# gbonneau-hardent/smallz4

Hardware: AMD Instinct MI355X
Metric: input MB/s at -9 optimal parse; output-byte diff vs smallz4 (must be 0) (higher is better)
Workload: dtype u8

## Files before the change

smallz4_amd/csrc/sz4_host.cpp:

```cpp
#include <hip/hip_runtime.h>

#include <algorithm>
#include <chrono>
#include <mutex>
#include <cstdio>
#include <atomic>
#include <cstring>
#include <string>
#include <new>
#include <vector>

#include "../../include/smallz4_amd.h"
#include "sz4_internal.h"
#include "sz4_mem.h"
#include "sz4_plan.h"

using namespace sz4;

namespace {

constexpr uint64_t kPad = 64;
constexpr uint64_t kBatchChunkDefault = 448ull << 20;
constexpr uint64_t kScratchPerByte = 50;
constexpr uint64_t kPieceFloor = 16ull << 20;
// ... 85 lines not shown
  PipeArgs a{};
  a.in = in;
  a.blocks = blocks.as<Block>();
  a.nblocks = (uint32_t)plan.blocks.size();
  a.segs = segs.as<Segment>();
  a.nsegs = (uint32_t)plan.segs.size();
  a.dpSegs = dpSegs.as<DpSeg>();
  a.ndp = (uint32_t)plan.dp.size();
  a.maxDpCount = plan.maxDpCount;
  a.walkSegs = walkSegs.as<uint2>();
  a.nwalk = (uint32_t)plan.walk.size();
  a.maxChain = maxChain;
  a.iv = iv.as<Interval>();
  a.ivCount = ivCount.as<uint32_t>();
  a.mlen = mlen.as<uint32_t>();
  a.mdist = mdist.as<uint16_t>();
  a.sel = sel();
  a.cost = cost.as<uint32_t>();
  a.reach = reach.as<uint32_t>();
  a.longFlag = longFlag.as<uint32_t>();
  a.longBits = longBits.as<uint32_t>();
  a.segLong = segLong.as<uint32_t>();
  a.segTail = segTail.as<uint64_t>();
  a.rank = rank.as<uint32_t>();
  const Plan::WorkOffsets& off = plan.off;
  a.elemA = work.as<uint2>();
  a.elemB = work_at<uint2>(off.elemB);
  a.rmqUp = work_at<uint32_t>(off.rmqUp);
  a.rmqDown = work_at<uint32_t>(off.rmqDown);
  a.dpSide = work_at<uint2>(off.side);
  a.dpRec = dpRec.as<uint4>();
  a.segState = segState.as<uint4>();
  a.lazySlots = work_at<uint32_t>(off.lazy);
  a.walkSlots = work_at<uint32_t>(off.walk);
  a.walkState = walkState.as<uint4>();
  a.tokens = work_at<Token>(off.tok);
  a.ntok = ntok.as<uint32_t>();
  a.blockBytes = blockBytes.as<uint32_t>();
  a.offsets = offsets.as<uint64_t>();
  a.status = status.as<int>();
  a.ldsWindow = plan.ldsWindow;
  a.out = out;
  a.headerLen = hdrLen;
  a.chosen = maxChain > (uint32_t)kGreedyMax ? a.sel : a.mlen;
  return a;
}

hipError_t Pipe::upload_plan(hipStream_t s) const
{
  hipError_t e = hipSuccess;
  (e = hipMemcpyAsync(blocks.p, plan.blocks.data(), plan.blocks.size() * sizeof(Block), hipMemcpyHostToDevice, s)) ||
      (e = hipMemcpyAsync(segs.p, plan.segs.data(), plan.segs.size() * sizeof(Segment), hipMemcpyHostToDevice, s)) ||
      (e = hipMemcpyAsync(dpSegs.p, plan.dp.data(), plan.dp.size() * sizeof(DpSeg), hipMemcpyHostToDevice, s)) ||
      (e = hipMemcpyAsync(walkSegs.p, plan.walk.data(), plan.walk.size() * sizeof(uint2), hipMemcpyHostToDevice, s));
  return e;
}

}

struct sz4_ctx {
  int device = 0;
  std::string err;
  bool timing = false;
  hipEvent_t ev[kStages + 1] = {};
  float stageMs[kStages] = {};
  uint32_t lastBlocks = 0;
  int stopAfter = 0;
  uint32_t lastChain = 0;

// ... 1703 lines not shown
```

smallz4_amd/csrc/sz4_internal.h:

```cpp
#pragma once
#include <stdint.h>

#include <hip/hip_runtime.h>

namespace sz4 {

constexpr int kMinMatch = 4;
constexpr int kTailNoMatch = 12;
constexpr int kTailLiterals = 5;
constexpr uint32_t kWindow = 65535;
constexpr uint32_t kSameLetter = 19 + 255 * 256;
constexpr int kGreedyMax = 3;
constexpr int kLazyMax = 6;
constexpr uint32_t kHashMul = 48271;
constexpr int kHashBits = 20;
constexpr uint64_t kNone = ~0ull;
constexpr uint32_t kRmqLen = 274;
constexpr uint32_t kFlagRmq = 1;
constexpr uint32_t kFlagRun = 2;
constexpr int kStages = 6;

constexpr int kStPrepRound = 2;
constexpr int kStInvariant = 4;

// ... 9 lines not shown
  uint32_t walkFirst;
  uint32_t walkCount;
  uint32_t dpSize;
  uint32_t pad;
};
constexpr uint32_t kNoBlock = 0xFFFFFFFFu;
constexpr uint32_t kBlkLegacy = 1;

struct Segment {
  uint64_t w0, s0, s1;
  uint64_t elemOff;
  uint64_t rankOff;
  uint32_t block;
  uint32_t pad;
};

struct Interval {
  uint64_t lo, hi;
  uint64_t a;
  uint64_t La;
};
constexpr uint32_t kMaxIv = 136;

struct DpSeg {
  uint32_t block;
  uint32_t k;
  uint32_t lo, hi;
};
inline uint32_t dp_segment_size(uint64_t n) { return n <= 65536 ? 4096u : 8192u; }
constexpr uint32_t kMaxDpSegs = 2048;

constexpr uint32_t kWalkSeg = 4096;
constexpr uint32_t kWalkCap = kWalkSeg / 4 + 2;

struct Token {
  uint32_t litFrom, lits, mlen, dist;
};
constexpr uint32_t kTokLast = 0x80000000u;

constexpr uint32_t kFindLds = 65536 + 16;
constexpr uint32_t find_lds_bytes() { return kFindLds; }
constexpr uint32_t kDpSide = 512;
constexpr uint32_t kDpSideKeys = kDpSide + 256;
constexpr uint32_t kDpSideStride = kDpSide + kDpSideKeys;
constexpr uint32_t dp_side_positions() { return kDpSideStride; }
constexpr uint32_t kLazyCap = 1400;
constexpr uint32_t lazy_slots_per_walk() { return 2 * kLazyCap; }

struct PipeArgs {
  const uint8_t* in;
  const Block* blocks;
  uint32_t nblocks;
  const Segment* segs;
  uint32_t nsegs;
  const DpSeg* dpSegs;
  uint32_t ndp;
  uint32_t maxDpCount;
  const uint2* walkSegs;
  uint32_t nwalk;
  uint32_t maxChain;
  Interval* iv;
  uint32_t* ivCount;
  uint32_t* mlen;
  uint16_t* mdist;
  uint32_t* sel;
  uint32_t* cost;
  uint32_t* reach;
  uint32_t* longFlag;
  uint32_t* longBits;
  uint32_t* segLong;
  uint64_t* segTail;
  uint32_t* rank;
  uint2* elemA;
  uint2* elemB;
  uint32_t* rmqUp;
  uint32_t* rmqDown;
  uint2* dpSide;
  uint4* dpRec;
  uint4* segState;
  uint32_t* lazySlots;
  uint32_t* walkSlots;
  uint4* walkState;
  Token* tokens;
  uint32_t* ntok;
  uint32_t* blockBytes;
  uint64_t* offsets;
  int* status;
  bool ldsWindow;
  uint8_t* out;
  uint64_t headerLen;
  const uint32_t* chosen;
};
void launch_runs(const PipeArgs& a, hipStream_t s);
void launch_find(int pass, const PipeArgs& a, hipStream_t s);
constexpr uint64_t kBlockMaxDict = 4ull << 20;
constexpr uint64_t kBlockMaxLegacy = 8ull << 20;
struct DictArgs : PipeArgs {
  const Block* hBlocks;
  uint32_t dictBack, cont, shift, low0;
  int legacy;
  uint32_t* last;
  uint16_t *prevH, *prevX, *ph, *pe;
  uint64_t *keysA, *keysB;
  void* temp;
  uint64_t tempBytes;
  uint32_t* lzMasks;
  uint64_t* scBits;
  uint2* runTab;
  uint32_t* runFlag;
  bool buildRuns;
  bool guess;
};
void launch_dict(const DictArgs& a, hipStream_t s);
uint64_t dict_sort_keys_max();
uint64_t dict_sort_temp_bytes();
uint64_t dict_sc_bits_bytes(uint32_t nb, uint64_t maxBlock);
// ... 102 lines not shown
```

smallz4_amd/csrc/sz4_kernels.hip:

```cpp
#include <hip/hip_runtime.h>
#include <stdint.h>
#include <stdlib.h>

#include <type_traits>

#include "sz4_internal.h"
#include "sz4_device.h"

#ifndef SZ4_SKIP_SHIFT
#define SZ4_SKIP_SHIFT 0
#endif
#ifndef SZ4_SKIP_BCAST
#define SZ4_SKIP_BCAST 0
#endif
#ifndef SZ4_SKIP_SEARCH
#define SZ4_SKIP_SEARCH 0
#endif
#ifndef SZ4_DIAG
#define SZ4_DIAG 0
#endif
#if SZ4_DIAG == 3
#define SZ4_D3(...) __VA_ARGS__
#else
#define SZ4_D3(...)
#endif
#if SZ4_DIAG == 5
#define SZ4_D5(...) __VA_ARGS__
#else
#define SZ4_D5(...)
#endif
#if SZ4_DIAG == 7
#define SZ4_D7(...) __VA_ARGS__
#else
#define SZ4_D7(...)
#endif

namespace sz4 {


__device__ __forceinline__ uint32_t lload4(const uint32_t* w, uint32_t off)
// ... 4797 lines not shown
        deltaTab[k] = convDelta;
        aboveTab[k] = 0;
        if (!done) segState[B.dpFirst + k] = make_uint4(lits, litBump, 0u, 0u);
      }
      prevV = convDelta;
      prevConv = (uint32_t)conv;
      prevDone = done;
      __syncthreads();
      prevKeyLim = convBlk[k];
    }
  }
  SZ4_D7(
  if (!kPar && lane == 0) {
    const uint64_t dt = __builtin_readcyclecounter() - d7t0;
    atomicAdd((unsigned long long*)&sz4_diag[0], (unsigned long long)d7Serial);
    atomicAdd((unsigned long long*)&sz4_diag[1], (unsigned long long)d7Closed);
    atomicAdd((unsigned long long*)&sz4_diag[2], (unsigned long long)d7Lit);
    atomicAdd((unsigned long long*)&sz4_diag[3], (unsigned long long)d7Segs);
    atomicMax((unsigned long long*)&sz4_diag[4], (unsigned long long)d7Serial);
    atomicAdd((unsigned long long*)&sz4_diag[5], (unsigned long long)dt);
    atomicMax((unsigned long long*)&sz4_diag[6], (unsigned long long)dt);
    atomicAdd((unsigned long long*)&sz4_diag[7], 1ull);
    if (rmq) atomicAdd((unsigned long long*)&sz4_diag[8], 1ull);
    for (int q = 0; q < 4; q++) atomicAdd((unsigned long long*)&sz4_diag[9 + q], (unsigned long long)d7Tk[q]);
  }
  )
}



__global__ __launch_bounds__(64 * kWalkWaves) void k_walk(const Block* __restrict__ blocks,
                                                          const uint2* __restrict__ walkSegs, uint32_t nwalk,
                                                          const uint32_t* __restrict__ chosen,
                                                          uint32_t* __restrict__ slotsAll, uint4* __restrict__ state,
                                                          int* __restrict__ status)
{
  const uint32_t wave = (uint32_t)__builtin_amdgcn_readfirstlane((int)(threadIdx.x >> 6));
  const uint32_t idx = blockIdx.x * kWalkWaves + wave;
  if (idx >= nwalk) return;
  const uint32_t lane = threadIdx.x & 63;
  const uint2 ws = walkSegs[idx];
  const Block B = blocks[ws.x];
  if (ws.y >= B.walkCount) return;
  const uint32_t n = (uint32_t)(B.end - B.start);
  const uint32_t* L = chosen + B.start;
  uint32_t* slots = slotsAll + (uint64_t)idx * (2 * kWalkCap) + kWalkCap;
  const uint32_t a = ws.y * kWalkSeg;
  const uint32_t aNext = a + kWalkSeg < n ? a + kWalkSeg : n;

  auto ldw = [&](uint32_t b) -> uint32_t {
    const uint32_t i = b + lane;
    return L[i < n ? i : n - 1u];
  };
  uint32_t wbase = a, e = 0, m = 0, exitPos = aNext;
  uint32_t wL = ldw(a), nL = ldw(a + 64);
  while (true) {
    const uint32_t lim = aNext - wbase < 64u ? aNext - wbase : 64u;
    const uint32_t len = wbase + lane < n && wL > 1u ? wL : 1u;
    const uint64_t mm = __ballot(len > 1u && lane >= e && lane < lim);
    uint32_t next, lastLen = 1;
    if (mm == 0) {
      next = wbase + lim;
    } else {
      const uint32_t x = wave_path(lane + len < 64u ? lane + len : 64u, e, lane);
      const bool rec = x == lane && len > 1u && lane < lim;
      const uint64_t rb = __ballot(rec);
      const uint32_t cnt = (uint32_t)__builtin_popcountll(rb);
      if (m + cnt > kWalkCap) {
        if (lane == 0) atomicOr(status, kStInvariant);
        break;
      }
      if (rec) slots[m + __builtin_amdgcn_mbcnt_hi((uint32_t)(rb >> 32), __builtin_amdgcn_mbcnt_lo((uint32_t)rb, 0u))] = wbase + lane;
      m += cnt;
      const uint32_t p = rdlane(x, lim - 1u);
      lastLen = rdlane(len, p);
      next = wbase + p + lastLen;
    }
    if (next >= aNext) {
      exitPos = lastLen > 1u ? next : aNext;
      break;
    }
    const uint32_t nb = next & ~63u;
    wL = nb == wbase + 64u ? nL : ldw(nb);
    nL = ldw(nb + 64u);
    wbase = nb;
    e = next & 63u;
  }
  if (lane == 0) state[idx] = make_uint4(kWalkCap, kWalkCap + m, exitPos, 0u);
}

struct WalkRepair {
  const uint32_t* L;
  const uint32_t* slots;
  uint32_t lane;
  __device__ __forceinline__ uint4 run(uint32_t* fix, uint32_t a, uint32_t aNext, uint4 st, uint32_t entry, int* status) const
  {
    const uint32_t m = st.y - kWalkCap;
    if (entry == a) return make_uint4(st.x, 0u, st.z, entry);
    if (entry >= aNext) return make_uint4(st.y, 0u, entry, entry);
    auto first_at = [&](uint32_t from, uint32_t p) -> uint32_t {
      for (uint32_t b = from; b < m; b += 64) {
        const uint64_t ge = __ballot(b + lane < m && slots[kWalkCap + b + lane] >= p);
        if (ge) return b + (uint32_t)__builtin_ctzll(ge);
      }
      return m;
    };
    auto inside = [&](uint32_t i, uint32_t q) -> bool {
      if (i == 0) return false;
      const uint32_t pj = slots[kWalkCap + i - 1];
      return pj + L[pj] > q;
    };
    uint32_t i = first_at(0, entry);
    if (!inside(i, entry)) return make_uint4(kWalkCap + i, 0u, st.z, entry);
    uint32_t q = entry, f = 0;
    bool merged = false;
    while (q < aNext) {
      const uint32_t lq = L[q];
      if (lq > 1u) {
        if (f >= kWalkCap) {
          if (lane == 0) atomicOr(status, kStInvariant);
          break;
        }
        if (lane == 0) fix[f] = q;
        f++;
        q += lq;
      } else {
        q++;
      }
      i = first_at(i, q);
      if (q < aNext && !inside(i, q)) {
        merged = true;
        break;
      }
    }
    const uint32_t iMerge = merged ? i : m;
    return make_uint4(kWalkCap + iMerge - f, f, merged ? st.z : q, entry);
  }
};

__global__ __launch_bounds__(64 * kWalkWaves) void k_walk_fix_spec(const Block* __restrict__ blocks,
                                                                   const uint2* __restrict__ walkSegs, uint32_t nwalk,
                                                                   const uint32_t* __restrict__ chosen,
                                                                   uint32_t* __restrict__ slotsAll,
                                                                   const uint4* __restrict__ state, uint4* __restrict__ rec,
                                                                   int* __restrict__ status)
{
  __shared__ uint32_t fixAll[kWalkWaves][kWalkCap];
  const uint32_t wave = (uint32_t)__builtin_amdgcn_readfirstlane((int)(threadIdx.x >> 6));
  const uint32_t idx = blockIdx.x * kWalkWaves + wave;
  if (idx >= nwalk) return;
  const uint2 ws = walkSegs[idx];
  if (ws.y == 0) return;
  const uint32_t lane = threadIdx.x & 63;
  const Block B = blocks[ws.x];
  if (ws.y >= B.walkCount) return;
  const uint32_t n = (uint32_t)(B.end - B.start);
  const uint32_t a = ws.y * kWalkSeg, aNext = a + kWalkSeg < n ? a + kWalkSeg : n;
  uint32_t* slots = slotsAll + (uint64_t)idx * (2 * kWalkCap);
  const WalkRepair W{chosen + B.start, slots, lane};
  uint32_t* fix = fixAll[wave];
  const uint4 r = W.run(fix, a, aNext, state[idx], state[idx - 1].z, status);
  __builtin_amdgcn_wave_barrier();
  for (uint32_t t = lane; t < r.y; t += 64) slots[t] = fix[t];
  if (lane == 0) rec[idx] = r;
}

__global__ __launch_bounds__(64) void k_walk_fix_commit(const Block* __restrict__ blocks, const uint32_t* __restrict__ chosen,
                                                        uint32_t* __restrict__ slotsAll,
                                                        uint4* __restrict__ state, const uint4* __restrict__ rec,
                                                        int* __restrict__ status)
{
  __shared__ uint32_t fix[kWalkCap];
  const Block B = blocks[blockIdx.x];
  if (B.walkCount < 2) return;
  const uint32_t lane = threadIdx.x;
  const uint32_t n = (uint32_t)(B.end - B.start);
  const uint32_t* L = chosen + B.start;
  uint32_t T = state[B.walkFirst].z;
  for (uint32_t k0 = 1; k0 < B.walkCount; k0 += 64) {
    const uint32_t cnt = B.walkCount - k0 < 64u ? B.walkCount - k0 : 64u;
    const uint32_t idxL = B.walkFirst + k0 + lane;
    const uint4 r = lane < cnt ? rec[idxL] : make_uint4(0, 0, 0, 0);
    uint32_t cur = 0;
    while (cur < cnt) {
      uint32_t prevExit = __shfl_up(r.z, 1, 64);
      if (lane == cur) prevExit = T;
      const uint64_t bad = __ballot(lane >= cur && lane < cnt && r.w != prevExit);
      const uint32_t js = bad ? (uint32_t)__builtin_ctzll(bad) : cnt;
      if (lane >= cur && lane < js) {
        uint32_t* slots = slotsAll + (uint64_t)idxL * (2 * kWalkCap);
        for (uint32_t t = r.y; t-- > 0;) slots[r.x + t] = slots[t];
        uint32_t* s32 = reinterpret_cast<uint32_t*>(state + idxL);
        s32[0] = r.x;
        s32[2] = r.z;
      }
      if (js == cnt) {
        T = rdlane(r.z, cnt - 1u);
        break;
      }
      const uint32_t idx = B.walkFirst + k0 + js;
      const uint32_t a = (k0 + js) * kWalkSeg, aNext = a + kWalkSeg < n ? a + kWalkSeg : n;
      uint32_t* slots = slotsAll + (uint64_t)idx * (2 * kWalkCap);
      const WalkRepair W{L, slots, lane};
      const uint4 st = state[idx];
      const uint4 rr = W.run(fix, a, aNext, st, rdlane(prevExit, js), status);
      __syncthreads();
      for (uint32_t t = lane; t < rr.y; t += 64) slots[rr.x + t] = fix[t];
      if (lane == 0) state[idx] = make_uint4(rr.x, st.y, rr.z, 0u);
      __syncthreads();
      T = rr.z;
      cur = js + 1;
    }
  }
}

__device__ __forceinline__ uint64_t token_bytes(uint64_t lits, uint32_t mlen, bool last)
{
  uint64_t b = 1 + lits + (lits >= 15 ? (lits - 15) / 255 + 1 : 0);
  if (!last) {
    const int64_t mcode = (int64_t)mlen - kMinMatch;
    b += 2 + (mcode >= 15 ? (uint64_t)(mcode - 15) / 255 + 1 : 0);
  }
  return b;
}

__global__ __launch_bounds__(1024) void k_scan(const uint32_t* __restrict__ blockBytes, uint32_t nblocks,
                                               uint64_t* __restrict__ offsets)
{
  __shared__ uint64_t s_carry;
  __shared__ uint32_t s_w[16];
  const uint32_t tid = threadIdx.x, lane = tid & 63, wave = tid >> 6;
  if (tid == 0) s_carry = 0;
  __syncthreads();
  for (uint32_t base = 0; base < nblocks; base += 1024) {
    const uint32_t i = base + tid;
    const uint32_t v = i < nblocks ? (blockBytes[i] & 0x7FFFFFFFu) : 0u;
    const uint32_t incl = wave_incl_scan_add(v);
    if (lane == 63) s_w[wave] = incl;
    __syncthreads();
    uint64_t pre = s_carry;
    for (uint32_t w = 0; w < wave; w++) pre += s_w[w];
    if (i < nblocks) offsets[i] = pre + incl - v;
    __syncthreads();
    if (tid == 1023) s_carry = pre + incl;
    __syncthreads();
  }
  if (tid == 0) offsets[nblocks] = s_carry;
}

constexpr uint64_t kOwnLits = 64;

constexpr int kAsmThreads = 1024;
constexpr int kSegWaves = 4;

__device__ __forceinline__ uint32_t wave_sum_u32(uint32_t v)
{
#pragma unroll
  for (int d = 32; d >= 1; d >>= 1) v += __shfl_xor(v, d, 64);
  return v;
}

__global__ __launch_bounds__(kAsmThreads) void k_seg_scan(const Block* __restrict__ blocks, const uint32_t* __restrict__ chosen,
                                                          const uint32_t* __restrict__ slotsAll,
                                                          const uint4* __restrict__ state, uint4* __restrict__ info)
{
  __shared__ uint32_t s_sum[kAsmThreads / 64], s_max[kAsmThreads / 64];
  const Block B = blocks[blockIdx.x];
  if (B.start == B.end) return;
  const uint32_t* L = chosen + B.start;
  const uint32_t tid = threadIdx.x, lane = tid & 63, wave = tid >> 6;
  uint32_t carrySum = 0, carryMax = 0;
  for (uint32_t k0 = 0; k0 < B.walkCount; k0 += kAsmThreads) {
    const uint32_t k = k0 + tid;
    const bool valid = k < B.walkCount;
    const uint32_t idx = B.walkFirst + k;
    uint32_t cnt = 0, lastEnd = 0;
    if (valid) {
      const uint4 st = state[idx];
      cnt = st.y - st.x;
      if (cnt) {
        const uint32_t p = slotsAll[(uint64_t)idx * (2 * kWalkCap) + st.y - 1];
        lastEnd = p + L[p];
      }
    }
    const uint32_t incS = wave_incl_scan_add(cnt), incM = wave_incl_scan_max(lastEnd);
    uint32_t prevM = __shfl_up(incM, 1, 64);
    if (lane == 0) prevM = 0;
    if (lane == 63) {
      s_sum[wave] = incS;
      s_max[wave] = incM;
    }
    __syncthreads();
    uint32_t preS = carrySum, preM = carryMax;
    for (uint32_t w = 0; w < wave; w++) {
      preS += s_sum[w];
      preM = s_max[w] > preM ? s_max[w] : preM;
    }
    if (valid) info[idx] = make_uint4(preS + incS - cnt, prevM > preM ? prevM : preM, 0u, 0u);
    for (uint32_t w = 0; w < kAsmThreads / 64; w++) {
      carrySum += s_sum[w];
      carryMax = s_max[w] > carryMax ? s_max[w] : carryMax;
    }
    __syncthreads();
  }
}

__global__ __launch_bounds__(64 * kSegWaves) void k_seg_tokens(const Block* __restrict__ blocks, const uint2* __restrict__ walkSegs,
                                                              uint32_t nwalk, const uint32_t* __restrict__ chosen,
                                                              const uint16_t* __restrict__ mdist,
                                                              const uint32_t* __restrict__ slotsAll, const uint4* __restrict__ state,
                                                              uint4* __restrict__ info, Token* __restrict__ tokAll,
                                                              uint2* __restrict__ blockTail)
{
  const uint32_t wave = (uint32_t)__builtin_amdgcn_readfirstlane((int)(threadIdx.x >> 6));
  const uint32_t idx = blockIdx.x * kSegWaves + wave;
  if (idx >= nwalk) return;
  const uint32_t lane = threadIdx.x & 63;
  const uint2 ws = walkSegs[idx];
  const Block B = blocks[ws.x];
  if (ws.y >= B.walkCount) return;
  const uint32_t n = (uint32_t)(B.end - B.start);
  const uint32_t* L = chosen + B.start;
  const uint16_t* D = mdist + B.start;
  const uint4 st = state[idx];
  const uint4 inf = info[idx];
  const uint32_t m = st.y - st.x;
  const uint32_t* slots = slotsAll + (uint64_t)idx * (2 * kWalkCap);
  Token* tok = tokAll + B.tokOff + inf.x;
  uint32_t carryEnd = inf.y, bytes = 0;
  uint32_t pN = lane < m ? slots[st.x + lane] : 0u;
  uint32_t LN = lane < m ? L[pN] : 0u, DN = lane < m ? (uint32_t)D[pN] : 0u;
  uint32_t pNN = 64u + lane < m ? slots[st.x + 64u + lane] : 0u;
  for (uint32_t c0 = 0; c0 < m; c0 += 64) {
    const uint32_t t = c0 + lane;
    const bool valid = t < m;
    uint32_t p, Lm, Dm;
    asm volatile("v_mov_b32 %0, %1" : "=v"(p) : "v"(pN));
    asm volatile("v_mov_b32 %0, %1" : "=v"(Lm) : "v"(LN));
    asm volatile("v_mov_b32 %0, %1" : "=v"(Dm) : "v"(DN));
    pN = pNN;
    LN = t + 64u < m ? L[pN] : 0u;
    DN = t + 64u < m ? (uint32_t)D[pN] : 0u;
    pNN = t + 128u < m ? slots[st.x + t + 128u] : 0u;
    const uint32_t end = p + Lm;
    uint32_t prev = __shfl_up(end, 1, 64);
    if (lane == 0) prev = carryEnd;
    uint32_t sz = 0;
    if (valid) {
      const uint32_t lits = p - prev;
      tok[t] = Token{lits ? prev : 0u, lits, Lm, Dm};
      sz = (uint32_t)token_bytes(lits, Lm, false);
    }
    bytes += wave_sum_u32(sz);
    carryEnd = rdlane(end, m - c0 < 64 ? m - c0 - 1 : 63);
  }
  if (lane == 0) info[idx].z = bytes;
  if (ws.y + 1 == B.walkCount && lane == 0) {
    const uint32_t M = inf.x + m;
    tokAll[B.tokOff + M] = Token{carryEnd, n - carryEnd, 0u, kTokLast};
    blockTail[ws.x] = make_uint2(M, (uint32_t)token_bytes(n - carryEnd, 0, true));
  }
}

__global__ __launch_bounds__(kAsmThreads) void k_block_bytes(const Block* __restrict__ blocks, uint32_t maxChain,
                                                             uint4* __restrict__ info, const uint2* __restrict__ blockTail,
                                                             uint32_t* __restrict__ ntokOut, uint32_t* __restrict__ blockBytes,
                                                             int* __restrict__ status)
{
  __shared__ uint32_t s_sum[kAsmThreads / 64];
  const Block B = blocks[blockIdx.x];
  const uint32_t tid = threadIdx.x, lane = tid & 63, wave = tid >> 6;
  const uint64_t n = B.end - B.start;
  if (n == 0) {
    if (tid == 0) ntokOut[blockIdx.x] = 0u, blockBytes[blockIdx.x] = 0u;
    return;
  }
  const bool stored = maxChain == 0;
  const bool legacy = (B.flags & kBlkLegacy) != 0;
  uint64_t enc = 0;
  uint32_t ntok = 0;
  if (!stored) {
    uint32_t carry = 0;
    for (uint32_t k0 = 0; k0 < B.walkCount; k0 += kAsmThreads) {
      const uint32_t k = k0 + tid;
      const bool valid = k < B.walkCount;
      const uint32_t idx = B.walkFirst + k;
      const uint32_t b = valid ? info[idx].z : 0u;
      const uint32_t inc = wave_incl_scan_add(b);
      if (lane == 63) s_sum[wave] = inc;
      __syncthreads();
      uint32_t pre = carry;
      for (uint32_t w = 0; w < wave; w++) pre += s_sum[w];
      if (valid) info[idx].w = pre + inc - b;
      for (uint32_t w = 0; w < kAsmThreads / 64; w++) carry += s_sum[w];
      __syncthreads();
    }
    const uint2 tail = blockTail[blockIdx.x];
    enc = (uint64_t)carry + tail.y;
    ntok = tail.x + 1;
  }
  const bool useEnc = (enc < n && !stored) || legacy;
  const uint32_t bytes = (uint32_t)(useEnc ? enc : n);
  if (tid == 0 && (ntok > n / 2 + 4 || (useEnc ? enc : n) >= 0x7FFFFFFBull)) atomicOr(status, kStInvariant);
  if (tid == 0) {
    ntokOut[blockIdx.x] = useEnc ? ntok : 0u;
    blockBytes[blockIdx.x] = (useEnc ? 0u : 0x80000000u) | (bytes + 4u);
  }
}

__global__ __launch_bounds__(64 * kSegWaves) void k_write_seg(const uint8_t* __restrict__ in, const Block* __restrict__ blocks,
                                                             const uint2* __restrict__ walkSegs, uint32_t nwalk,
                                                             const uint4* __restrict__ state, const uint4* __restrict__ info,
                                                             const Token* __restrict__ tokAll, const uint32_t* __restrict__ ntokAll,
                                                             const uint32_t* __restrict__ blockBytes,
                                                             const uint64_t* __restrict__ offsets, uint8_t* __restrict__ out,
                                                             uint64_t headerLen)
{
  __shared__ uint32_t s_ld[kSegWaves][64], s_ls[kSegWaves][64], s_ll[kSegWaves][64];
  const uint32_t wave = (uint32_t)__builtin_amdgcn_readfirstlane((int)(threadIdx.x >> 6));
  const uint32_t idx = blockIdx.x * kSegWaves + wave;
  if (idx >= nwalk) return;
  const uint32_t lane = threadIdx.x & 63;
  const uint2 ws = walkSegs[idx];
  const Block B = blocks[ws.x];
  if (ws.y >= B.walkCount) return;
  const uint64_t n = B.end - B.start;
  const uint32_t bb = blockBytes[ws.x];
  const bool raw = (bb & 0x80000000u) != 0;
  uint8_t* dst = out + headerLen + offsets[ws.x];
  if (ws.y == 0 && lane == 0) {
    const uint32_t word = ((bb & 0x7FFFFFFFu) - 4u) | (raw ? 0x80000000u : 0u);
    dst[0] = (uint8_t)word;
    dst[1] = (uint8_t)(word >> 8);
    dst[2] = (uint8_t)(word >> 16);
    dst[3] = (uint8_t)(word >> 24);
  }
  dst += 4;
  const uint8_t* src = in + B.start;
  if (raw) {
    const uint64_t lo = (uint64_t)ws.y * kWalkSeg, hi = lo + kWalkSeg < n ? lo + kWalkSeg : n;
    for (uint64_t j = lo + lane; j < hi; j += 64) dst[j] = src[j];
    return;
  }
  if (ntokAll[ws.x] == 0) return;
  const uint4 st = state[idx], inf = info[idx];
  const uint32_t count = (st.y - st.x) + (ws.y + 1 == B.walkCount ? 1u : 0u);
  const Token* tok = tokAll + B.tokOff + inf.x;
  uint64_t carry = inf.w;
  for (uint32_t c0 = 0; c0 < count; c0 += 64) {
    const uint32_t t = c0 + lane;
    const bool valid = t < count;
    Token T{0, 0, 0, 0};
    uint64_t sz = 0;
    bool last = false;
    if (valid) {
      T = tok[t];
      last = (T.dist & kTokLast) != 0;
      sz = token_bytes(T.lits, T.mlen, last);
    }
    uint64_t incl = sz;
#pragma unroll
    for (int d = 1; d < 64; d <<= 1) {
      const uint64_t o = __shfl_up(incl, d, 64);
      if (lane >= (uint32_t)d) incl += o;
    }
    const uint64_t off = carry + incl - sz;
    carry += __shfl(incl, 63, 64);
    bool isLong = false;
    if (valid) {
      uint8_t* o = dst + off;
      const int64_t mcode = last ? 0 : (int64_t)T.mlen - kMinMatch;
      const uint8_t tk = (uint8_t)(mcode < 15 ? mcode : 15);
      const uint64_t lits = T.lits;
      if (lits < 15) {
        *o++ = (uint8_t)(tk | (lits << 4));
      } else {
        *o++ = (uint8_t)(tk | 0xF0);
        uint64_t v = lits - 15;
        while (v >= 255) { *o++ = 255; v -= 255; }
        *o++ = (uint8_t)v;
      }
      if (lits <= kOwnLits) {
        for (uint32_t k = 0; k < (uint32_t)lits; k += 8) {
          const uint64_t a = (uint64_t)T.litFrom + k;
          const uint32_t nk = (uint32_t)lits - k < 8u ? (uint32_t)lits - k : 8u;
          const uintptr_t ab = reinterpret_cast<uintptr_t>(src + a);
          if (a >= 4u && a + 12u <= n) {
            const uint32_t* wp = reinterpret_cast<const uint32_t*>(ab & ~(uintptr_t)3);
            const uint32_t w0 = wp[0], w1 = wp[1], w2 = wp[2];
            const uint32_t sh = (uint32_t)(ab & 3u);
            const uint32_t v0 = __builtin_amdgcn_alignbyte(w1, w0, sh), v1 = __builtin_amdgcn_alignbyte(w2, w1, sh);
#pragma unroll
// ... 109 lines not shown
  hipMemsetAsync(firstBad, 0xFF, (size_t)a.nblocks * 4, s);
  hipLaunchKernelGGL(k_lazy_check, walks, walkBlock, 0, s, a.in, a.blocks, a.walkSegs, a.nwalk, a.iv, a.ivCount, a.longFlag,
                     a.mlen, a.mdist, a.lazySlots, a.walkState, firstBad);
  hipLaunchKernelGGL(k_lazy_correct, dim3(a.nblocks), dim3(64), 0, s, a.blocks, a.iv, a.ivCount, a.mlen, firstBad,
                     a.status);
}

void launch_parse(const PipeArgs& a, hipStream_t s)
{
  if (!a.nblocks) return;
  if (a.maxChain <= (uint32_t)kGreedyMax || !a.ndp) return;
  const dim3 specGrid((a.ndp + kSpecWaves - 1) / kSpecWaves), specBlock(64 * kSpecWaves);
  hipLaunchKernelGGL(k_dp_spec_lean, specGrid, specBlock, 0, s, a.blocks, a.dpSegs, a.ndp, a.mlen, a.mdist, a.cost, a.sel,
                     a.reach, a.segState, a.longFlag, a.rmqUp, a.rmqDown);
  hipLaunchKernelGGL(k_dp_spec_rmq, specGrid, specBlock, 0, s, a.blocks, a.dpSegs, a.ndp, a.mlen, a.mdist, a.cost, a.sel,
                     a.reach, a.segState, a.longFlag, a.rmqUp, a.rmqDown);
  hipLaunchKernelGGL(k_dp_fix<true>, dim3(a.ndp), dim3(64), 0, s, a.blocks, a.dpSegs, a.ndp, a.mlen, a.mdist, a.cost, a.sel,
                     a.reach, a.segState, a.longFlag, a.rmqUp, a.rmqDown, a.dpSide, a.dpRec, 0u);
  const uint32_t tab = a.maxDpCount < 1u ? 1u : a.maxDpCount > kMaxDpSegs ? kMaxDpSegs : a.maxDpCount;
  hipLaunchKernelGGL(k_dp_fix<false>, dim3(a.nblocks), dim3(64), 4 * tab * sizeof(uint32_t), s, a.blocks, a.dpSegs, a.ndp,
                     a.mlen, a.mdist, a.cost, a.sel, a.reach, a.segState, a.longFlag, a.rmqUp, a.rmqDown, a.dpSide, a.dpRec,
                     tab);
}

void launch_emit(const PipeArgs& a, hipStream_t s)
{
  if (!a.nblocks) return;
  const bool walk = a.maxChain > 0 && a.nwalk;
  const dim3 walks((a.nwalk + kWalkWaves - 1) / kWalkWaves), walkBlock(64 * kWalkWaves);
  const dim3 segGrid((a.nwalk + kSegWaves - 1) / kSegWaves), segBlock(64 * kSegWaves);
  uint4* info = reinterpret_cast<uint4*>(a.reach);
  uint2* blockTail = reinterpret_cast<uint2*>(info + a.nwalk);
  if (walk) {
    hipLaunchKernelGGL(k_walk, walks, walkBlock, 0, s, a.blocks, a.walkSegs, a.nwalk, a.chosen, a.walkSlots, a.walkState,
                       a.status);
    hipLaunchKernelGGL(k_walk_fix_spec, walks, walkBlock, 0, s, a.blocks, a.walkSegs, a.nwalk, a.chosen, a.walkSlots,
                       a.walkState, info, a.status);
    hipLaunchKernelGGL(k_walk_fix_commit, dim3(a.nblocks), dim3(64), 0, s, a.blocks, a.chosen, a.walkSlots, a.walkState,
                       info, a.status);
    hipLaunchKernelGGL(k_seg_scan, dim3(a.nblocks), dim3(kAsmThreads), 0, s, a.blocks, a.chosen, a.walkSlots, a.walkState,
                       info);
    hipLaunchKernelGGL(k_seg_tokens, segGrid, segBlock, 0, s, a.blocks, a.walkSegs, a.nwalk, a.chosen, a.mdist, a.walkSlots,
                       a.walkState, info, a.tokens, blockTail);
  }
  hipLaunchKernelGGL(k_block_bytes, dim3(a.nblocks), dim3(kAsmThreads), 0, s, a.blocks, a.maxChain, info, blockTail, a.ntok,
                     a.blockBytes, a.status);
  hipLaunchKernelGGL(k_scan, dim3(1), dim3(1024), 0, s, a.blockBytes, a.nblocks, a.offsets);
  if (a.nwalk)
    hipLaunchKernelGGL(k_write_seg, segGrid, segBlock, 0, s, a.in, a.blocks, a.walkSegs, a.nwalk, a.walkState, info, a.tokens,
                       a.ntok, a.blockBytes, a.offsets, a.out, a.headerLen);
}

}
```

smallz4_amd/csrc/sz4_plan.cpp:

```cpp
#include "sz4_plan.h"

#include <stdlib.h>

#include <algorithm>

namespace sz4 {

Block independent_block(uint64_t start, uint64_t end, uint32_t flags)
{
  Block B{};
  B.start = start;
  B.end = end;
  B.low = start;
  B.cut = kNone;
  B.prev = kNoBlock;
  B.flags = flags;
  return B;
}

bool Plan::begin(const PlanKey& k)
{
  if (k == key) return false;
  key = PlanKey{};
  blocks.clear();
// ... 57 lines not shown
    }
    B.dpSize = (uint32_t)seg;
    for (uint64_t hi = top, i = 0;; hi -= seg, i++) {
      const uint64_t lo = hi + 1 >= seg ? hi + 1 - seg : 0;
      dp.push_back(DpSeg{b, (uint32_t)i, (uint32_t)lo, (uint32_t)hi});
      B.dpCount++;
      if (lo == 0) break;
    }
    maxDpCount = std::max(maxDpCount, B.dpCount);
  }
  ldsWindow = true;
  for (const Segment& S : segs) {
    const Block& B = blocks[S.block];
    if ((B.end - S.w0 + 8 + 3) / 4 * 4 > find_lds_bytes()) ldsWindow = false;
  }
  key = k;
}

uint64_t Plan::work_layout(uint64_t stagedBytes)
{
  auto al = [](uint64_t b) { return (b + 255) & ~255ull; };
  const uint64_t nb = blocks.size();
  const uint64_t elem = al(elemTotal * sizeof(uint2) + 64);
  off.elemB = elem;
  const uint64_t findEnd = 2 * elem;
  const uint64_t selBytes = al(stagedBytes * 4 + 64), rmq = al((stagedBytes + nb + 8) * 4);
  off.rmqUp = selBytes;
  off.rmqDown = selBytes + rmq;
  off.side = selBytes + 2 * rmq;
  const uint64_t parseEnd = off.side + al(dp.size() * dp_side_positions() * sizeof(uint2) + 64);
  off.lazy = selBytes;
  const uint64_t lazyEnd = off.lazy + al(walk.size() * lazy_slots_per_walk() * 4ull + 64);
  off.tok = selBytes;
  off.walk = off.tok + al(tokTotal * sizeof(Token) + 64);
  const uint64_t emitEnd = off.walk + al(walk.size() * 2 * kWalkCap * 4 + 64);
  return std::max(std::max(findEnd, parseEnd), std::max(lazyEnd, emitEnd));
}

void Plan::build_uniform(uint64_t len, uint32_t blockSize)
{
  const PlanKey k{PlanKey::kUniform, len, blockSize};
  if (!begin(k)) return;
  for (uint64_t st = 0; st < len; st += blockSize)
    blocks.push_back(independent_block(st, std::min<uint64_t>(st + blockSize, len)));
  finish_plan(k);
}

void Plan::build_stream(uint64_t pre, uint64_t n, bool first, int legacy, bool dictMode)
{
  const PlanKey k{PlanKey::kStream, 0, 0, pre, n, first, legacy, dictMode};
  if (!begin(k)) return;
  const uint64_t bs = legacy ? kBlockMaxLegacy : kBlockMaxDict;
  for (uint64_t st = 0; st < n; st += bs) {
    Block B = independent_block(pre + st, pre + std::min(st + bs, n), legacy ? kBlkLegacy : 0);
    if (!legacy && !(st == 0 && first)) {
      B.low = B.start - kWindow;
      B.cut = B.start - kTailNoMatch;
      B.prev = st == 0 ? kNoBlock - 1 : (uint32_t)blocks.size() - 1;
    }
    blocks.push_back(B);
  }
  const uint32_t nb = (uint32_t)blocks.size();
  if (nb && blocks[0].prev == kNoBlock - 1) blocks[0].prev = nb;
  finish_plan(k);
}

uint64_t Plan::build_ragged(const std::vector<uint64_t>& sizes)
// ... 58 lines not shown
```

Before: 15610.

## Pack match records into 64-bit walk slots and drop the token array

Walk slots now hold packed 64-bit records (position, length, distance) instead of bare positions, so later stages no longer gather L[p] and D[p] through a position indirection. The separate Token array and its write in the segment pass are removed, and the writer rebuilds literal spans from neighbouring records with shuffles. The spec-fix kernel writes repairs straight into global slots instead of LDS, and slots are laid out per block via tokOff with per-segment caps. This trades wider slot storage and a 24-bit position/length limit for fewer global writes and random reads.

```diff
diff --git a/smallz4_amd/csrc/sz4_host.cpp b/smallz4_amd/csrc/sz4_host.cpp
--- a/smallz4_amd/csrc/sz4_host.cpp
+++ b/smallz4_amd/csrc/sz4_host.cpp
@@ -141,9 +141,8 @@
   a.dpRec = dpRec.as<uint4>();
   a.segState = segState.as<uint4>();
   a.lazySlots = work_at<uint32_t>(off.lazy);
-  a.walkSlots = work_at<uint32_t>(off.walk);
+  a.walkSlots = work_at<uint64_t>(off.tok);
   a.walkState = walkState.as<uint4>();
-  a.tokens = work_at<Token>(off.tok);
   a.ntok = ntok.as<uint32_t>();
   a.blockBytes = blockBytes.as<uint32_t>();
   a.offsets = offsets.as<uint64_t>();
diff --git a/smallz4_amd/csrc/sz4_internal.h b/smallz4_amd/csrc/sz4_internal.h
--- a/smallz4_amd/csrc/sz4_internal.h
+++ b/smallz4_amd/csrc/sz4_internal.h
@@ -65,11 +65,8 @@
 
 constexpr uint32_t kWalkSeg = 4096;
 constexpr uint32_t kWalkCap = kWalkSeg / 4 + 2;
-
-struct Token {
-  uint32_t litFrom, lits, mlen, dist;
-};
-constexpr uint32_t kTokLast = 0x80000000u;
+constexpr uint32_t walk_cap(uint32_t r) { return r / 4 + 2 < kWalkCap ? r / 4 + 2 : kWalkCap; }
+constexpr uint64_t walk_slot_first(uint64_t tokOff, uint32_t k) { return 2 * tokOff + (uint64_t)k * kWalkSeg; }
 
 constexpr uint32_t kFindLds = 65536 + 16;
 constexpr uint32_t find_lds_bytes() { return kFindLds; }
@@ -112,9 +109,8 @@
   uint4* dpRec;
   uint4* segState;
   uint32_t* lazySlots;
-  uint32_t* walkSlots;
+  uint64_t* walkSlots;
   uint4* walkState;
-  Token* tokens;
   uint32_t* ntok;
   uint32_t* blockBytes;
   uint64_t* offsets;
diff --git a/smallz4_amd/csrc/sz4_kernels.hip b/smallz4_amd/csrc/sz4_kernels.hip
--- a/smallz4_amd/csrc/sz4_kernels.hip
+++ b/smallz4_amd/csrc/sz4_kernels.hip
@@ -6,6 +6,7 @@
 
 #include "sz4_internal.h"
 #include "sz4_device.h"
+#include "sz4_match_rec.h"
 
 #ifndef SZ4_SKIP_SHIFT
 #define SZ4_SKIP_SHIFT 0
@@ -4869,7 +4870,8 @@
 __global__ __launch_bounds__(64 * kWalkWaves) void k_walk(const Block* __restrict__ blocks,
                                                           const uint2* __restrict__ walkSegs, uint32_t nwalk,
                                                           const uint32_t* __restrict__ chosen,
-                                                          uint32_t* __restrict__ slotsAll, uint4* __restrict__ state,
+                                                          const uint16_t* __restrict__ mdist,
+                                                          uint64_t* __restrict__ slotsAll, uint4* __restrict__ state,
                                                           int* __restrict__ status)
 {
   const uint32_t wave = (uint32_t)__builtin_amdgcn_readfirstlane((int)(threadIdx.x >> 6));
@@ -4881,16 +4883,23 @@
   if (ws.y >= B.walkCount) return;
   const uint32_t n = (uint32_t)(B.end - B.start);
   const uint32_t* L = chosen + B.start;
-  uint32_t* slots = slotsAll + (uint64_t)idx * (2 * kWalkCap) + kWalkCap;
+  const uint16_t* D = mdist + B.start;
   const uint32_t a = ws.y * kWalkSeg;
   const uint32_t aNext = a + kWalkSeg < n ? a + kWalkSeg : n;
+  const uint32_t cap = walk_cap(aNext - a);
+  uint64_t* slots = slotsAll + walk_slot_first(B.tokOff, ws.y) + cap;
 
   auto ldw = [&](uint32_t b) -> uint32_t {
     const uint32_t i = b + lane;
     return L[i < n ? i : n - 1u];
   };
+  auto ldd = [&](uint32_t b) -> uint32_t {
+    const uint32_t i = b + lane;
+    return D[i < n ? i : n - 1u];
+  };
   uint32_t wbase = a, e = 0, m = 0, exitPos = aNext;
   uint32_t wL = ldw(a), nL = ldw(a + 64);
+  uint32_t wD = ldd(a), nD = ldd(a + 64);
   while (true) {
     const uint32_t lim = aNext - wbase < 64u ? aNext - wbase : 64u;
     const uint32_t len = wbase + lane < n && wL > 1u ? wL : 1u;
@@ -4903,11 +4912,13 @@
       const bool rec = x == lane && len > 1u && lane < lim;
       const uint64_t rb = __ballot(rec);
       const uint32_t cnt = (uint32_t)__builtin_popcountll(rb);
-      if (m + cnt > kWalkCap) {
+      if (m + cnt > cap) {
         if (lane == 0) atomicOr(status, kStInvariant);
         break;
       }
-      if (rec) slots[m + __builtin_amdgcn_mbcnt_hi((uint32_t)(rb >> 32), __builtin_amdgcn_mbcnt_lo((uint32_t)rb, 0u))] = wbase + lane;
+      if (rec)
+        slots[m + __builtin_amdgcn_mbcnt_hi((uint32_t)(rb >> 32), __builtin_amdgcn_mbcnt_lo((uint32_t)rb, 0u))] =
+            mrec_pack(wbase + lane, len, wD);
       m += cnt;
       const uint32_t p = rdlane(x, lim - 1u);
       lastLen = rdlane(len, p);
@@ -4919,46 +4930,49 @@
     }
     const uint32_t nb = next & ~63u;
     wL = nb == wbase + 64u ? nL : ldw(nb);
+    wD = nb == wbase + 64u ? nD : ldd(nb);
     nL = ldw(nb + 64u);
+    nD = ldd(nb + 64u);
     wbase = nb;
     e = next & 63u;
   }
-  if (lane == 0) state[idx] = make_uint4(kWalkCap, kWalkCap + m, exitPos, 0u);
+  if (lane == 0) state[idx] = make_uint4(cap, cap + m, exitPos, 0u);
 }
 
 struct WalkRepair {
   const uint32_t* L;
-  const uint32_t* slots;
+  const uint16_t* D;
+  const uint64_t* slots;
   uint32_t lane;
-  __device__ __forceinline__ uint4 run(uint32_t* fix, uint32_t a, uint32_t aNext, uint4 st, uint32_t entry, int* status) const
+  uint32_t cap;
+  __device__ __forceinline__ uint4 run(uint64_t* fix, uint32_t a, uint32_t aNext, uint4 st, uint32_t entry, int* status) const
   {
-    const uint32_t m = st.y - kWalkCap;
+    const uint32_t m = st.y - cap;
     if (entry == a) return make_uint4(st.x, 0u, st.z, entry);
     if (entry >= aNext) return make_uint4(st.y, 0u, entry, entry);
     auto first_at = [&](uint32_t from, uint32_t p) -> uint32_t {
       for (uint32_t b = from; b < m; b += 64) {
-        const uint64_t ge = __ballot(b + lane < m && slots[kWalkCap + b + lane] >= p);
+        const uint64_t ge = __ballot(b + lane < m && mrec_pos(slots[cap + b + lane]) >= p);
         if (ge) return b + (uint32_t)__builtin_ctzll(ge);
       }
       return m;
     };
     auto inside = [&](uint32_t i, uint32_t q) -> bool {
       if (i == 0) return false;
-      const uint32_t pj = slots[kWalkCap + i - 1];
-      return pj + L[pj] > q;
+      return mrec_end(slots[cap + i - 1]) > q;
     };
     uint32_t i = first_at(0, entry);
-    if (!inside(i, entry)) return make_uint4(kWalkCap + i, 0u, st.z, entry);
+    if (!inside(i, entry)) return make_uint4(cap + i, 0u, st.z, entry);
     uint32_t q = entry, f = 0;
     bool merged = false;
     while (q < aNext) {
       const uint32_t lq = L[q];
       if (lq > 1u) {
-        if (f >= kWalkCap) {
+        if (f >= cap) {
           if (lane == 0) atomicOr(status, kStInvariant);
           break;
         }
-        if (lane == 0) fix[f] = q;
+        if (lane == 0) fix[f] = mrec_pack(q, lq, D[q]);
         f++;
         q += lq;
       } else {
@@ -4971,18 +4985,18 @@
       }
     }
     const uint32_t iMerge = merged ? i : m;
-    return make_uint4(kWalkCap + iMerge - f, f, merged ? st.z : q, entry);
+    return make_uint4(cap + iMerge - f, f, merged ? st.z : q, entry);
   }
 };
 
 __global__ __launch_bounds__(64 * kWalkWaves) void k_walk_fix_spec(const Block* __restrict__ blocks,
                                                                    const uint2* __restrict__ walkSegs, uint32_t nwalk,
                                                                    const uint32_t* __restrict__ chosen,
-                                                                   uint32_t* __restrict__ slotsAll,
+                                                                   const uint16_t* __restrict__ mdist,
+                                                                   uint64_t* __restrict__ slotsAll,
                                                                    const uint4* __restrict__ state, uint4* __restrict__ rec,
                                                                    int* __restrict__ status)
 {
-  __shared__ uint32_t fixAll[kWalkWaves][kWalkCap];
   const uint32_t wave = (uint32_t)__builtin_amdgcn_readfirstlane((int)(threadIdx.x >> 6));
   const uint32_t idx = blockIdx.x * kWalkWaves + wave;
   if (idx >= nwalk) return;
@@ -4993,26 +5007,25 @@
   if (ws.y >= B.walkCount) return;
   const uint32_t n = (uint32_t)(B.end - B.start);
   const uint32_t a = ws.y * kWalkSeg, aNext = a + kWalkSeg < n ? a + kWalkSeg : n;
-  uint32_t* slots = slotsAll + (uint64_t)idx * (2 * kWalkCap);
-  const WalkRepair W{chosen + B.start, slots, lane};
-  uint32_t* fix = fixAll[wave];
-  const uint4 r = W.run(fix, a, aNext, state[idx], state[idx - 1].z, status);
-  __builtin_amdgcn_wave_barrier();
-  for (uint32_t t = lane; t < r.y; t += 64) slots[t] = fix[t];
+  uint64_t* slots = slotsAll + walk_slot_first(B.tokOff, ws.y);
+  const WalkRepair W{chosen + B.start, mdist + B.start, slots, lane, walk_cap(aNext - a)};
+  const uint4 r = W.run(slots, a, aNext, state[idx], state[idx - 1].z, status);
   if (lane == 0) rec[idx] = r;
 }
 
 __global__ __launch_bounds__(64) void k_walk_fix_commit(const Block* __restrict__ blocks, const uint32_t* __restrict__ chosen,
-                                                        uint32_t* __restrict__ slotsAll,
+                                                        const uint16_t* __restrict__ mdist,
+                                                        uint64_t* __restrict__ slotsAll,
                                                         uint4* __restrict__ state, const uint4* __restrict__ rec,
                                                         int* __restrict__ status)
 {
-  __shared__ uint32_t fix[kWalkCap];
+  __shared__ uint64_t fix[kWalkCap];
   const Block B = blocks[blockIdx.x];
   if (B.walkCount < 2) return;
   const uint32_t lane = threadIdx.x;
   const uint32_t n = (uint32_t)(B.end - B.start);
   const uint32_t* L = chosen + B.start;
+  const uint16_t* D = mdist + B.start;
   uint32_t T = state[B.walkFirst].z;
   for (uint32_t k0 = 1; k0 < B.walkCount; k0 += 64) {
     const uint32_t cnt = B.walkCount - k0 < 64u ? B.walkCount - k0 : 64u;
@@ -5025,7 +5038,7 @@
       const uint64_t bad = __ballot(lane >= cur && lane < cnt && r.w != prevExit);
       const uint32_t js = bad ? (uint32_t)__builtin_ctzll(bad) : cnt;
       if (lane >= cur && lane < js) {
-        uint32_t* slots = slotsAll + (uint64_t)idxL * (2 * kWalkCap);
+        uint64_t* slots = slotsAll + walk_slot_first(B.tokOff, k0 + lane);
         for (uint32_t t = r.y; t-- > 0;) slots[r.x + t] = slots[t];
         uint32_t* s32 = reinterpret_cast<uint32_t*>(state + idxL);
         s32[0] = r.x;
@@ -5037,8 +5050,8 @@
       }
       const uint32_t idx = B.walkFirst + k0 + js;
       const uint32_t a = (k0 + js) * kWalkSeg, aNext = a + kWalkSeg < n ? a + kWalkSeg : n;
-      uint32_t* slots = slotsAll + (uint64_t)idx * (2 * kWalkCap);
-      const WalkRepair W{L, slots, lane};
+      uint64_t* slots = slotsAll + walk_slot_first(B.tokOff, k0 + js);
+      const WalkRepair W{L, D, slots, lane, walk_cap(aNext - a)};
       const uint4 st = state[idx];
       const uint4 rr = W.run(fix, a, aNext, st, rdlane(prevExit, js), status);
       __syncthreads();
@@ -5049,16 +5062,6 @@
       cur = js + 1;
     }
   }
-}
-
-__device__ __forceinline__ uint64_t token_bytes(uint64_t lits, uint32_t mlen, bool last)
-{
-  uint64_t b = 1 + lits + (lits >= 15 ? (lits - 15) / 255 + 1 : 0);
-  if (!last) {
-    const int64_t mcode = (int64_t)mlen - kMinMatch;
-    b += 2 + (mcode >= 15 ? (uint64_t)(mcode - 15) / 255 + 1 : 0);
-  }
-  return b;
 }
 
 __global__ __launch_bounds__(1024) void k_scan(const uint32_t* __restrict__ blockBytes, uint32_t nblocks,
@@ -5097,14 +5100,13 @@
   return v;
 }
 
-__global__ __launch_bounds__(kAsmThreads) void k_seg_scan(const Block* __restrict__ blocks, const uint32_t* __restrict__ chosen,
-                                                          const uint32_t* __restrict__ slotsAll,
+__global__ __launch_bounds__(kAsmThreads) void k_seg_scan(const Block* __restrict__ blocks,
+                                                          const uint64_t* __restrict__ slotsAll,
                                                           const uint4* __restrict__ state, uint4* __restrict__ info)
 {
   __shared__ uint32_t s_sum[kAsmThreads / 64], s_max[kAsmThreads / 64];
   const Block B = blocks[blockIdx.x];
   if (B.start == B.end) return;
-  const uint32_t* L = chosen + B.start;
   const uint32_t tid = threadIdx.x, lane = tid & 63, wave = tid >> 6;
   uint32_t carrySum = 0, carryMax = 0;
   for (uint32_t k0 = 0; k0 < B.walkCount; k0 += kAsmThreads) {
@@ -5115,10 +5117,7 @@
     if (valid) {
       const uint4 st = state[idx];
       cnt = st.y - st.x;
-      if (cnt) {
-        const uint32_t p = slotsAll[(uint64_t)idx * (2 * kWalkCap) + st.y - 1];
-        lastEnd = p + L[p];
-      }
+      if (cnt) lastEnd = mrec_end(slotsAll[walk_slot_first(B.tokOff, k) + st.y - 1]);
     }
     const uint32_t incS = wave_incl_scan_add(cnt), incM = wave_incl_scan_max(lastEnd);
     uint32_t prevM = __shfl_up(incM, 1, 64);
@@ -5142,12 +5141,10 @@
   }
 }
 
-__global__ __launch_bounds__(64 * kSegWaves) void k_seg_tokens(const Block* __restrict__ blocks, const uint2* __restrict__ walkSegs,
-                                                              uint32_t nwalk, const uint32_t* __restrict__ chosen,
-                                                              const uint16_t* __restrict__ mdist,
-                                                              const uint32_t* __restrict__ slotsAll, const uint4* __restrict__ state,
-                                                              uint4* __restrict__ info, Token* __restrict__ tokAll,
-                                                              uint2* __restrict__ blockTail)
+__global__ __launch_bounds__(64 * kSegWaves) void k_seg_sizes(const Block* __restrict__ blocks, const uint2* __restrict__ walkSegs,
+                                                             uint32_t nwalk, const uint64_t* __restrict__ slotsAll,
+                                                             const uint4* __restrict__ state, uint4* __restrict__ info,
+                                                             uint2* __restrict__ blockTail)
 {
   const uint32_t wave = (uint32_t)__builtin_amdgcn_readfirstlane((int)(threadIdx.x >> 6));
   const uint32_t idx = blockIdx.x * kSegWaves + wave;
@@ -5157,45 +5154,26 @@
   const Block B = blocks[ws.x];
   if (ws.y >= B.walkCount) return;
   const uint32_t n = (uint32_t)(B.end - B.start);
-  const uint32_t* L = chosen + B.start;
-  const uint16_t* D = mdist + B.start;
   const uint4 st = state[idx];
   const uint4 inf = info[idx];
   const uint32_t m = st.y - st.x;
-  const uint32_t* slots = slotsAll + (uint64_t)idx * (2 * kWalkCap);
-  Token* tok = tokAll + B.tokOff + inf.x;
+  const uint64_t* recs = slotsAll + walk_slot_first(B.tokOff, ws.y) + st.x;
   uint32_t carryEnd = inf.y, bytes = 0;
-  uint32_t pN = lane < m ? slots[st.x + lane] : 0u;
-  uint32_t LN = lane < m ? L[pN] : 0u, DN = lane < m ? (uint32_t)D[pN] : 0u;
-  uint32_t pNN = 64u + lane < m ? slots[st.x + 64u + lane] : 0u;
+  uint64_t rN = lane < m ? recs[lane] : 0ull;
   for (uint32_t c0 = 0; c0 < m; c0 += 64) {
     const uint32_t t = c0 + lane;
-    const bool valid = t < m;
-    uint32_t p, Lm, Dm;
-    asm volatile("v_mov_b32 %0, %1" : "=v"(p) : "v"(pN));
-    asm volatile("v_mov_b32 %0, %1" : "=v"(Lm) : "v"(LN));
-    asm volatile("v_mov_b32 %0, %1" : "=v"(Dm) : "v"(DN));
-    pN = pNN;
-    LN = t + 64u < m ? L[pN] : 0u;
-    DN = t + 64u < m ? (uint32_t)D[pN] : 0u;
-    pNN = t + 128u < m ? slots[st.x + t + 128u] : 0u;
-    const uint32_t end = p + Lm;
+    const uint64_t r = rN;
+    rN = t + 64u < m ? recs[t + 64u] : 0ull;
+    const uint32_t p = mrec_pos(r), Lm = mrec_len(r), end = p + Lm;
     uint32_t prev = __shfl_up(end, 1, 64);
     if (lane == 0) prev = carryEnd;
-    uint32_t sz = 0;
-    if (valid) {
-      const uint32_t lits = p - prev;
-      tok[t] = Token{lits ? prev : 0u, lits, Lm, Dm};
-      sz = (uint32_t)token_bytes(lits, Lm, false);
-    }
-    bytes += wave_sum_u32(sz);
+    if (t < m) bytes += (uint32_t)token_bytes(p - prev, Lm, false);
     carryEnd = rdlane(end, m - c0 < 64 ? m - c0 - 1 : 63);
   }
+  bytes = wave_sum_u32(bytes);
   if (lane == 0) info[idx].z = bytes;
   if (ws.y + 1 == B.walkCount && lane == 0) {
-    const uint32_t M = inf.x + m;
-    tokAll[B.tokOff + M] = Token{carryEnd, n - carryEnd, 0u, kTokLast};
-    blockTail[ws.x] = make_uint2(M, (uint32_t)token_bytes(n - carryEnd, 0, true));
+    blockTail[ws.x] = make_uint2(inf.x + m, (uint32_t)token_bytes(n - carryEnd, 0, true));
   }
 }
 
@@ -5248,7 +5226,7 @@
 __global__ __launch_bounds__(64 * kSegWaves) void k_write_seg(const uint8_t* __restrict__ in, const Block* __restrict__ blocks,
                                                              const uint2* __restrict__ walkSegs, uint32_t nwalk,
                                                              const uint4* __restrict__ state, const uint4* __restrict__ info,
-                                                             const Token* __restrict__ tokAll, const uint32_t* __restrict__ ntokAll,
+                                                             const uint64_t* __restrict__ slotsAll, const uint32_t* __restrict__ ntokAll,
                                                              const uint32_t* __restrict__ blockBytes,
                                                              const uint64_t* __restrict__ offsets, uint8_t* __restrict__ out,
                                                              uint64_t headerLen)
@@ -5281,20 +5259,24 @@
   }
   if (ntokAll[ws.x] == 0) return;
   const uint4 st = state[idx], inf = info[idx];
-  const uint32_t count = (st.y - st.x) + (ws.y + 1 == B.walkCount ? 1u : 0u);
-  const Token* tok = tokAll + B.tokOff + inf.x;
+  const uint32_t m = st.y - st.x;
+  const uint32_t count = m + (ws.y + 1 == B.walkCount ? 1u : 0u);
+  const uint64_t* recs = slotsAll + walk_slot_first(B.tokOff, ws.y) + st.x;
   uint64_t carry = inf.w;
+  uint32_t carryEnd = inf.y;
   for (uint32_t c0 = 0; c0 < count; c0 += 64) {
     const uint32_t t = c0 + lane;
     const bool valid = t < count;
-    Token T{0, 0, 0, 0};
-    uint64_t sz = 0;
-    bool last = false;
-    if (valid) {
-      T = tok[t];
-      last = (T.dist & kTokLast) != 0;
-      sz = token_bytes(T.lits, T.mlen, last);
-    }
+    const bool last = valid && t == m;
+    const uint64_t r = t < m ? recs[t] : 0ull;
+    const uint32_t end = mrec_end(r);
+    uint32_t litFrom = __shfl_up(end, 1, 64);
+    if (lane == 0) litFrom = carryEnd;
+    if (m > c0) carryEnd = rdlane(end, m - c0 < 64 ? m - c0 - 1 : 63);
+    const struct {
+      uint32_t litFrom, lits, mlen, dist;
+    } T{litFrom, (last ? (uint32_t)n : mrec_pos(r)) - litFrom, mrec_len(r), mrec_dist(r)};
+    const uint64_t sz = valid ? token_bytes(T.lits, T.mlen, last) : 0;
     uint64_t incl = sz;
 #pragma unroll
     for (int d = 1; d < 64; d <<= 1) {
@@ -5470,22 +5452,21 @@
   uint4* info = reinterpret_cast<uint4*>(a.reach);
   uint2* blockTail = reinterpret_cast<uint2*>(info + a.nwalk);
   if (walk) {
-    hipLaunchKernelGGL(k_walk, walks, walkBlock, 0, s, a.blocks, a.walkSegs, a.nwalk, a.chosen, a.walkSlots, a.walkState,
-                       a.status);
-    hipLaunchKernelGGL(k_walk_fix_spec, walks, walkBlock, 0, s, a.blocks, a.walkSegs, a.nwalk, a.chosen, a.walkSlots,
+    hipLaunchKernelGGL(k_walk, walks, walkBlock, 0, s, a.blocks, a.walkSegs, a.nwalk, a.chosen, a.mdist, a.walkSlots,
+                       a.walkState, a.status);
+    hipLaunchKernelGGL(k_walk_fix_spec, walks, walkBlock, 0, s, a.blocks, a.walkSegs, a.nwalk, a.chosen, a.mdist, a.walkSlots,
                        a.walkState, info, a.status);
-    hipLaunchKernelGGL(k_walk_fix_commit, dim3(a.nblocks), dim3(64), 0, s, a.blocks, a.chosen, a.walkSlots, a.walkState,
-                       info, a.status);
-    hipLaunchKernelGGL(k_seg_scan, dim3(a.nblocks), dim3(kAsmThreads), 0, s, a.blocks, a.chosen, a.walkSlots, a.walkState,
-                       info);
-    hipLaunchKernelGGL(k_seg_tokens, segGrid, segBlock, 0, s, a.blocks, a.walkSegs, a.nwalk, a.chosen, a.mdist, a.walkSlots,
-                       a.walkState, info, a.tokens, blockTail);
+    hipLaunchKernelGGL(k_walk_fix_commit, dim3(a.nblocks), dim3(64), 0, s, a.blocks, a.chosen, a.mdist, a.walkSlots,
+                       a.walkState, info, a.status);
+    hipLaunchKernelGGL(k_seg_scan, dim3(a.nblocks), dim3(kAsmThreads), 0, s, a.blocks, a.walkSlots, a.walkState, info);
+    hipLaunchKernelGGL(k_seg_sizes, segGrid, segBlock, 0, s, a.blocks, a.walkSegs, a.nwalk, a.walkSlots, a.walkState, info,
+                       blockTail);
   }
   hipLaunchKernelGGL(k_block_bytes, dim3(a.nblocks), dim3(kAsmThreads), 0, s, a.blocks, a.maxChain, info, blockTail, a.ntok,
                      a.blockBytes, a.status);
   hipLaunchKernelGGL(k_scan, dim3(1), dim3(1024), 0, s, a.blockBytes, a.nblocks, a.offsets);
   if (a.nwalk)
-    hipLaunchKernelGGL(k_write_seg, segGrid, segBlock, 0, s, a.in, a.blocks, a.walkSegs, a.nwalk, a.walkState, info, a.tokens,
+    hipLaunchKernelGGL(k_write_seg, segGrid, segBlock, 0, s, a.in, a.blocks, a.walkSegs, a.nwalk, a.walkState, info, a.walkSlots,
                        a.ntok, a.blockBytes, a.offsets, a.out, a.headerLen);
 }
 
diff --git a/smallz4_amd/csrc/sz4_match_rec.h b/smallz4_amd/csrc/sz4_match_rec.h
--- /dev/null
+++ b/smallz4_amd/csrc/sz4_match_rec.h
@@ -0,0 +1,36 @@
+#pragma once
+#include <stdint.h>
+
+#ifdef __HIP__
+#define SZ4_REC_HD __host__ __device__
+#else
+#define SZ4_REC_HD
+#endif
+
+namespace sz4 {
+
+constexpr uint32_t kRecPosBits = 24, kRecLenBits = 24, kRecDistBits = 16;
+constexpr uint32_t kRecMask24 = (1u << 24) - 1u;
+
+SZ4_REC_HD inline uint64_t mrec_pack(uint32_t pos, uint32_t len, uint32_t dist)
+{
+  return (uint64_t)(pos & kRecMask24) | ((uint64_t)(len & kRecMask24) << kRecPosBits) |
+         ((uint64_t)(dist & 0xFFFFu) << (kRecPosBits + kRecLenBits));
+}
+SZ4_REC_HD inline uint32_t mrec_pos(uint64_t r) { return (uint32_t)r & kRecMask24; }
+SZ4_REC_HD inline uint32_t mrec_len(uint64_t r) { return (uint32_t)(r >> kRecPosBits) & kRecMask24; }
+SZ4_REC_HD inline uint32_t mrec_dist(uint64_t r) { return (uint32_t)(r >> (kRecPosBits + kRecLenBits)); }
+SZ4_REC_HD inline uint32_t mrec_end(uint64_t r) { return mrec_pos(r) + mrec_len(r); }
+
+constexpr int kRecMinMatch = 4;
+SZ4_REC_HD inline uint64_t token_bytes(uint64_t lits, uint32_t mlen, bool last)
+{
+  uint64_t b = 1 + lits + (lits >= 15 ? (lits - 15) / 255 + 1 : 0);
+  if (!last) {
+    const int64_t mcode = (int64_t)mlen - kRecMinMatch;
+    b += 2 + (mcode >= 15 ? (uint64_t)(mcode - 15) / 255 + 1 : 0);
+  }
+  return b;
+}
+
+}
diff --git a/smallz4_amd/csrc/sz4_plan.cpp b/smallz4_amd/csrc/sz4_plan.cpp
--- a/smallz4_amd/csrc/sz4_plan.cpp
+++ b/smallz4_amd/csrc/sz4_plan.cpp
@@ -113,7 +113,7 @@
   off.lazy = selBytes;
   const uint64_t lazyEnd = off.lazy + al(walk.size() * lazy_slots_per_walk() * 4ull + 64);
   off.tok = selBytes;
-  off.walk = off.tok + al(tokTotal * sizeof(Token) + 64);
+  off.walk = off.tok + al(tokTotal * 16 + 64);
   const uint64_t emitEnd = off.walk + al(walk.size() * 2 * kWalkCap * 4 + 64);
   return std::max(std::max(findEnd, parseEnd), std::max(lazyEnd, emitEnd));
 }
```

New measurement: 15980, median of 6. 2.3% higher.
